# HKUST-Aerial-Robotics/FUEL

Hardware: NVIDIA H100
Metric: replans_per_sec (higher is better)
Workload: dtype f64 (cost/gradient), i32+f32 (ESDF), u8 (frontier)

## Files before the change

fuel_b200/csrc/frontier.cu:

```cuda
#include "common.cuh"

#include <cooperative_groups.h>

#include <algorithm>
#include <vector>

namespace cg = cooperative_groups;

namespace {

constexpr int NONE = 0x7fffffff;

struct FParams {
  int dom_lo[3], dom_n[3];
  int s_lo[3], s_hi[3];
  int z_min_idx;
  int cluster_min;
  double size_xy;
  float leaf, leaf_inv;
};

__device__ __forceinline__ int tri_at(const Geom& g, const uint8_t* __restrict__ occ, int x, int y,
                                      int z) {
  if (x < 0 || y < 0 || z < 0 || x >= g.nx || y >= g.ny || z >= g.nz) return -1;
// ... 962 lines not shown
  }
  if (threadIdx.x == 0) *n_new = carry;
}

__device__ __forceinline__ void relabel_item(Geom g, const int* __restrict__ k_addr, int* __restrict__ k_cl,
                               const ClusterMeta* __restrict__ meta, int K, int C_old, int _tid) {
  const int k = _tid;
  if (k >= K) return;
  const int c = k_cl[k];
  if (c >= C_old || !meta[c].do_split) return;
  if (cell_side(g, meta[c], k_addr[k]) == 1) k_cl[k] = meta[c].new_id;
}

__device__ __forceinline__ void clear_do_split_item(ClusterMeta* meta, int C, int _tid) {
  const int c = _tid;
  if (c < C) meta[c].do_split = 0;
}

__device__ __forceinline__ void init_meta_item(ClusterMeta* meta, int R, int _tid) {
  const int c = _tid;
  if (c >= R) return;
  ClusterMeta m;
  memset(&m, 0, sizeof(m));
  m.root = c;
  m.active = 1;
  meta[c] = m;
}

__global__ void init_parent_kernel(int* parent, int* claim, int* csize, int n) {
  init_parent_item(parent, claim, csize, n, blockIdx.x * blockDim.x + threadIdx.x);
}

__global__ void union_kernel(Geom g, const int* __restrict__ cell_addr,
                             const uint8_t* __restrict__ cell_cls, const int* __restrict__ cellidx,
                             int* parent, int n) {
  union_item(g, cell_addr, cell_cls, cellidx, parent, n, blockIdx.x * blockDim.x + threadIdx.x);
}

__global__ void flatten_kernel(int* parent, const uint8_t* __restrict__ cell_cls, int n) {
  flatten_item(parent, cell_cls, n, blockIdx.x * blockDim.x + threadIdx.x);
}

__global__ void claim_kernel(Geom g, FParams fp, const int* __restrict__ cell_addr,
                             const uint8_t* __restrict__ cell_cls, const int* __restrict__ cellidx,
                             const int* __restrict__ label, int* claim, int n) {
  claim_item(g, fp, cell_addr, cell_cls, cellidx, label, claim, n, blockIdx.x * blockDim.x + threadIdx.x);
}

__global__ void assign_kernel(const int* __restrict__ cell_addr, const uint8_t* __restrict__ cell_cls,
                              const int* __restrict__ label, const int* __restrict__ claim,
                              int* __restrict__ seed, int* csize, int8_t* __restrict__ flag, int n) {
  assign_item(cell_addr, cell_cls, label, claim, seed, csize, flag, n, blockIdx.x * blockDim.x + threadIdx.x);
}

__global__ void mark_kernel(const int* __restrict__ seed, const int* __restrict__ csize, int cluster_min,
                            int* __restrict__ is_root, int* __restrict__ is_kept, int n) {
  mark_item(seed, csize, cluster_min, is_root, is_kept, n, blockIdx.x * blockDim.x + threadIdx.x);
}

__global__ void reset_cellidx_kernel(const int* __restrict__ cell_addr, int* __restrict__ cellidx, int n) {
  reset_cellidx_item(cell_addr, cellidx, n, blockIdx.x * blockDim.x + threadIdx.x);
}

__global__ void gather_kept_kernel(const int* __restrict__ cell_addr, const int* __restrict__ seed,
                                   const int* __restrict__ is_kept, const int* __restrict__ kept_off,
                                   const int* __restrict__ root_rank, int* __restrict__ k_addr,
                                   int* __restrict__ k_cl, int* __restrict__ cellidx, int n) {
  gather_kept_item(cell_addr, seed, is_kept, kept_off, root_rank, k_addr, k_cl, cellidx, n, blockIdx.x * blockDim.x + threadIdx.x);
}

struct LevelCtl {
  const int* R;
  const int* K;
  int* n_new;
  int* c_final;
  int* ccur;
  int* cnext;
};

__global__ void stat_accum_kernel(Geom g, const int* __restrict__ k_addr, const int* __restrict__ k_cl,
                                  const ClusterMeta* __restrict__ meta, ClusterStat* st, LevelCtl ctl) {
  if (*ctl.n_new == 0) return;
  stat_accum_item(g, k_addr, k_cl, meta, st, *ctl.K, blockIdx.x * blockDim.x + threadIdx.x);
}

__global__ void downsample_kernel(Geom g, FParams fp, const int* __restrict__ k_addr,
                                  const int* __restrict__ k_cl, const int* __restrict__ cellidx,
                                  const ClusterMeta* __restrict__ meta, ClusterStat* st,
                                  float* __restrict__ k_cent, int* __restrict__ k_leaf, LevelCtl ctl) {
  if (*ctl.n_new == 0) return;
  downsample_item<true>(g, fp, k_addr, k_cl, cellidx, meta, st, k_cent, k_leaf, *ctl.K, blockIdx.x * blockDim.x + threadIdx.x);
}

__global__ void cov_kernel(Geom g, const int* __restrict__ k_cl, const int* __restrict__ k_leaf,
                           const float* __restrict__ k_cent, const ClusterMeta* __restrict__ meta,
                           ClusterStat* st, LevelCtl ctl) {
  if (*ctl.n_new == 0) return;
  cov_item<true>(g, k_cl, k_leaf, k_cent, meta, st, *ctl.K, blockIdx.x * blockDim.x + threadIdx.x);
}

__global__ void pca_kernel(Geom g, ClusterMeta* meta, const ClusterStat* __restrict__ st, LevelCtl ctl) {
  if (*ctl.n_new == 0) return;
  const int c = blockIdx.x * blockDim.x + threadIdx.x;
  mean_item(g, meta, st, *ctl.ccur, c);
  pca_item(meta, st, *ctl.ccur, c);
}

__global__ void side_count_kernel(Geom g, const int* __restrict__ k_addr, const int* __restrict__ k_cl,
                                  const ClusterMeta* __restrict__ meta, ClusterStat* st, LevelCtl ctl) {
  if (*ctl.n_new == 0) return;
  side_count_item(g, k_addr, k_cl, meta, st, *ctl.K, blockIdx.x * blockDim.x + threadIdx.x);
}

__global__ void __launch_bounds__(1024) split_alloc_kernel(ClusterMeta* meta, const ClusterStat* __restrict__ st,
                                                           LevelCtl ctl) {
  if (*ctl.n_new == 0) return;
  const int C = *ctl.ccur;
  __shared__ int made;
  split_alloc(meta, st, C, &made);
  __syncthreads();
  if (threadIdx.x == 0) {
    *ctl.cnext = C + made;
    *ctl.c_final = C + made;
    *ctl.n_new = made;
  }
}

__global__ void relabel_kernel(Geom g, const int* __restrict__ k_addr, int* __restrict__ k_cl,
                               const ClusterMeta* __restrict__ meta, LevelCtl ctl) {
  if (*ctl.n_new == 0) return;
  relabel_item(g, k_addr, k_cl, meta, *ctl.K, *ctl.ccur, blockIdx.x * blockDim.x + threadIdx.x);
}

__global__ void next_level_kernel(ClusterMeta* meta, ClusterStat* st, LevelCtl ctl) {
  if (*ctl.n_new == 0) return;
  const int c = blockIdx.x * blockDim.x + threadIdx.x;
  clear_do_split_item(meta, *ctl.ccur, c);
  stat_reset_item(st, meta, *ctl.cnext, c);
}

__global__ void init_meta_kernel(ClusterMeta* meta, ClusterStat* st, LevelCtl ctl) {
  const int R = *ctl.R;
  const int c = blockIdx.x * blockDim.x + threadIdx.x;
  init_meta_item(meta, R, c);
  stat_reset_item(st, meta, R, c);
  if (c == 0) {
    *ctl.ccur = R;
    *ctl.c_final = R;
    *ctl.n_new = (R > 0 && *ctl.K > 0) ? 1 : 0;
  }
}


constexpr int SMALL_CTAS = 8;
constexpr int SMALL_CAP = 32768;
constexpr int SMALL_CCAP = 8192;


__device__ __forceinline__ void mark_chunk_item(const int* __restrict__ seed, const int* __restrict__ csize, int cluster_min,
                                                int* __restrict__ root_mask, int* __restrict__ kept_mask, int n, int i) {
  bool kept = false, root = false;
  if (i < n) {
    const int s = seed[i];
    kept = s != NONE && csize[s] > cluster_min;
    root = kept && s == i;
  }
  const unsigned mk = __ballot_sync(0xffffffffu, kept), mr = __ballot_sync(0xffffffffu, root);
  if ((i & 31) == 0 && i < n) {
    kept_mask[i >> 5] = (int)mk;
    root_mask[i >> 5] = (int)mr;
  }
}
__device__ void chunk_scan_small(const int* __restrict__ root_mask, const int* __restrict__ kept_mask,
                                 int* __restrict__ root_off, int* __restrict__ kept_off, int nchunk,
                                 int* __restrict__ tot_root, int* __restrict__ tot_kept) {
  __shared__ unsigned wtot2[32];
  const int t = threadIdx.x, lane = t & 31, w = t >> 5;
  const unsigned v = t < nchunk ? ((unsigned)__popc((unsigned)root_mask[t]) << 16) + (unsigned)__popc((unsigned)kept_mask[t]) : 0u;
  unsigned inc = v;
#pragma unroll
  for (int o = 1; o < 32; o <<= 1) {
    const unsigned u = __shfl_up_sync(0xffffffffu, inc, o);
    if (lane >= o) inc += u;
  }
  if (lane == 31) wtot2[w] = inc;
  __syncthreads();
  if (w == 0) {
    const unsigned x = wtot2[lane];
    unsigned xi = x;
#pragma unroll
    for (int o = 1; o < 32; o <<= 1) {
      const unsigned u = __shfl_up_sync(0xffffffffu, xi, o);
      if (lane >= o) xi += u;
    }
    wtot2[lane] = xi - x;
    if (lane == 31) {
      *tot_root = (int)(xi >> 16);
      *tot_kept = (int)(xi & 0xffffu);
    }
  }
  __syncthreads();
  if (t < nchunk) {
    const unsigned ex = wtot2[w] + inc - v;
    root_off[t] = (int)(ex >> 16);
    kept_off[t] = (int)(ex & 0xffffu);
  }
}
__device__ __forceinline__ void gather_chunk_item(const int* __restrict__ cell_addr, const int* __restrict__ seed,
                                                  const int* __restrict__ kept_mask, const int* __restrict__ kept_off,
                                                  const int* __restrict__ root_mask, const int* __restrict__ root_off,
                                                  int* __restrict__ k_addr, int* __restrict__ k_cl,
                                                  int* __restrict__ cellidx, int n, int i) {
  if (i >= n) return;
  const unsigned mk = (unsigned)kept_mask[i >> 5];
  const int a = cell_addr[i];
  if ((mk >> (i & 31)) & 1u) {
    const int k = kept_off[i >> 5] + __popc(mk & ((1u << (i & 31)) - 1u));
    const int s = seed[i];
    k_addr[k] = a;
    k_cl[k] = root_off[s >> 5] + __popc((unsigned)root_mask[s >> 5] & ((1u << (s & 31)) - 1u));
    cellidx[a] = k;
  } else {
    cellidx[a] = -1;
  }
}

struct SmallBufs {
  int *cell_addr, *parent, *claim, *csize, *seed, *is_root, *is_kept, *root_rank, *kept_off;
  uint8_t* cell_cls;
  int *k_addr, *k_cl, *k_leaf;
  float* k_cent;
  ClusterMeta* meta;
  ClusterStat* stat;
  int* counters;
};

__global__ void __cluster_dims__(SMALL_CTAS, 1, 1) __launch_bounds__(1024) cluster_small_kernel(Geom g, FParams fp, int8_t* __restrict__ flag,
                                                             int* __restrict__ cellidx, SmallBufs b) {
  cg::cluster_group cluster = cg::this_cluster();
  const int rank = (int)cluster.block_rank();
  const int tid = (((int)threadIdx.x >> 5) * SMALL_CTAS + rank) * 32 + ((int)threadIdx.x & 31);
  constexpr int NT = 1024 * SMALL_CTAS;
  const int n = b.counters[0];
#ifdef FUEL_PROF
  long long* prof = (long long*)(b.counters + 8);
  int pi = 0;
#define STAMP() do { if (tid == 0) { long long t_; asm volatile("mov.u64 %0, %%globaltimer;" : "=l"(t_)); prof[pi++] = t_; } } while (0)
#else
#define STAMP() do {} while (0)
#endif
  STAMP();
  if (n > SMALL_CAP) {
    if (tid == 0) b.counters[4] = 1;
    return;
  }
#define FOR_ITEMS(i, N) for (int i = tid; i - tid < (N); i += NT)
  FOR_ITEMS(i, n) init_parent_item(b.parent, b.claim, b.csize, n, i);
  cluster.sync();
  STAMP();
  FOR_ITEMS(i, n) union_item(g, b.cell_addr, b.cell_cls, cellidx, b.parent, n, i);
  cluster.sync();
  STAMP();
  FOR_ITEMS(i, n) flatten_item(b.parent, b.cell_cls, n, i);
  cluster.sync();
  STAMP();
  FOR_ITEMS(i, n) claim_item(g, fp, b.cell_addr, b.cell_cls, cellidx, b.parent, b.claim, n, i);
  cluster.sync();
  STAMP();
  FOR_ITEMS(i, n) assign_item(b.cell_addr, b.cell_cls, b.parent, b.claim, b.seed, b.csize, flag, n, i);
  cluster.sync();
  STAMP();
  FOR_ITEMS(i, n) mark_chunk_item(b.seed, b.csize, fp.cluster_min, b.is_root, b.is_kept, n, i);
  cluster.sync();
  STAMP();
  if (rank == 0) chunk_scan_small(b.is_root, b.is_kept, b.root_rank, b.kept_off, (n + 31) >> 5, b.counters + 1, b.counters + 2);
  cluster.sync();
  STAMP();
  const int R = b.counters[1], K = b.counters[2];
  int C = R;
  int status = 0;
  if (R > 0 && K > 0) {
    FOR_ITEMS(i, n) gather_chunk_item(b.cell_addr, b.seed, b.is_kept, b.kept_off, b.is_root, b.root_rank, b.k_addr, b.k_cl,
                                      cellidx, n, i);
    FOR_ITEMS(c, R) {
      init_meta_item(b.meta, R, c);
      stat_reset_item(b.stat, b.meta, R, c);
    }
    cluster.sync();
    STAMP();
    for (int level = 0; level < 40; ++level) {
      if (2 * C > SMALL_CCAP) {
        status = 2;
        break;
      }
      FOR_ITEMS(k, K) stat_accum_item(g, b.k_addr, b.k_cl, b.meta, b.stat, K, k);
      cluster.sync();
      STAMP();
      FOR_ITEMS(c, C) mean_item(g, b.meta, b.stat, C, c);
      FOR_ITEMS(k, K) downsample_item<true>(g, fp, b.k_addr, b.k_cl, cellidx, b.meta, b.stat, b.k_cent, b.k_leaf, K, k);
      cluster.sync();
      STAMP();
      FOR_ITEMS(k, K) cov_item(g, b.k_cl, b.k_leaf, b.k_cent, b.meta, b.stat, K, k);
      cluster.sync();
      STAMP();
      FOR_ITEMS(c, C) pca_item(b.meta, b.stat, C, c);
      cluster.sync();
      STAMP();
      FOR_ITEMS(k, K) side_count_item(g, b.k_addr, b.k_cl, b.meta, b.stat, K, k);
      cluster.sync();
      STAMP();
      if (rank == 0) split_alloc(b.meta, b.stat, C, b.counters + 3);
      cluster.sync();
      STAMP();
      FOR_ITEMS(k, K) relabel_item(g, b.k_addr, b.k_cl, b.meta, K, C, k);
      cluster.sync();
      STAMP();
      const int n_new = b.counters[3];
      if (n_new == 0) break;
      FOR_ITEMS(c, C) clear_do_split_item(b.meta, C, c);
      C += n_new;
      FOR_ITEMS(c, C) stat_reset_item(b.stat, b.meta, C, c);
      cluster.sync();
      STAMP();
    }
  }
  FOR_ITEMS(i, n) reset_cellidx_item(b.cell_addr, cellidx, n, i);
  if (tid == 0) {
    b.counters[4] = status;
    b.counters[5] = C;
  }
#undef FOR_ITEMS
}

__global__ void is_changed_kernel(Geom g, const uint8_t* __restrict__ occ, const int* __restrict__ offs,
                                  const int* __restrict__ addr, uint8_t* __restrict__ changed, int* __restrict__ counts,
                                  int m) {
  const int c = blockIdx.x;
  if (c >= m) return;
  __shared__ int cnt;
  if (threadIdx.x == 0) cnt = 0;
  __syncthreads();
  int mine = 0;
  for (int i = offs[c] + threadIdx.x; i < offs[c + 1]; i += blockDim.x) {
    int x, y, z;
    addr_to_idx(g, addr[i], x, y, z);
    if (!frontier_pred(g, occ, x, y, z)) ++mine;
  }
  if (mine) atomicAdd(&cnt, mine);
  __syncthreads();
  if (threadIdx.x == 0) {
    if (changed) changed[c] = (uint8_t)(cnt > 0);
    if (counts) counts[c] = cnt;
  }
}

template <typename T>
struct DevBuf {
  T* p = nullptr;
  size_t cap = 0;
  int ensure(size_t n) {
    if (n <= cap) return 0;
    if (p) cudaFree(p);
    p = nullptr;
    cap = 0;
    size_t want = n + n / 4 + 1024;
    if (cudaMalloc(&p, want * sizeof(T)) != cudaSuccess) return FUELGPU_ENOMEM;
    cap = want;
    return 0;
  }
  int grow_preserve(size_t n, size_t keep, cudaStream_t s) {
    if (n <= cap) return 0;
    T* np = nullptr;
    size_t want = n + n / 2 + 1024;
    if (cudaMalloc(&np, want * sizeof(T)) != cudaSuccess) return FUELGPU_ENOMEM;
    if (p && keep) {
      cudaMemcpyAsync(np, p, keep * sizeof(T), cudaMemcpyDeviceToDevice, s);
      cudaStreamSynchronize(s);
    }
    if (p) cudaFree(p);
    p = np;
    cap = want;
    return 0;
  }
  void release() {
    if (p) cudaFree(p);
    p = nullptr;
    cap = 0;
  }
};

}

struct SweepPlan {
  bool words = false;
  unsigned nb = 0;
  size_t nmask = 0;
  int64_t ndom = 0;
  WordGeom wg;
};

struct HostView {
  const int *addr, *cl, *leaf;
  const float* cent;
  const ClusterMeta* meta;
  const ClusterStat* stat;
};

struct FrontierState {
  int* cellidx = nullptr;
  DevBuf<uint32_t> maskE, maskS;
  DevBuf<int> blockcnt, blockoff, scan_tot, scan_off;
  DevBuf<int> cell_addr, parent, claim, csize, seed, is_root, is_kept, root_rank, kept_off;
  DevBuf<uint8_t> cell_cls;
  DevBuf<int> k_addr, k_cl, k_leaf;
  DevBuf<float> k_cent;
  DevBuf<ClusterStat> stat;
  DevBuf<ClusterMeta> meta;
  bool small_ready = false;
  bool pend_active = false, pend_empty = true;
  FParams pend_fp;
  SweepPlan pend_plan;
  HostView pend_hv;
  cudaStream_t stream = nullptr;
  cudaEvent_t ev_in = nullptr;
  cudaEvent_t ev_out = nullptr;
  bool ev_out_valid = false;
  char* h_pin = nullptr;
  size_t h_pin_bytes = 0;
  int* d_counters = nullptr;
  std::vector<int32_t> h_cell_off, h_cell_addr, h_filt_off;
  std::vector<double> h_filtered, h_avg, h_bmin, h_bmax;
  int cell_order = FUELGPU_CELLS_BY_ADDRESS;
  float last_leaf = 0.f;
};

cudaStream_t frontier_stream_raw(FuelMap* m) { return m->fs->stream; }
cudaStream_t frontier_stream(FuelMap* m) {
  FrontierState* f = m->fs;
  cudaEventRecord(f->ev_in, m->stream);
  cudaStreamWaitEvent(f->stream, f->ev_in, 0);
  return f->stream;
}

int frontier_set_cell_order(FuelMap* m, int order) {
  if (order != FUELGPU_CELLS_BY_ADDRESS && order != FUELGPU_CELLS_BFS)
    return fuel_fail(m, FUELGPU_EINVAL, "unknown cell order");
  m->fs->cell_order = order;
  return 0;
}

void frontier_order_writer(FuelMap* m) {
  FrontierState* f = m->fs;
  if (f && f->ev_out_valid) cudaStreamWaitEvent(m->stream, f->ev_out, 0);
}

int frontier_state_create(FuelMap* m) {
  m->fs = new FrontierState();
  FUEL_CUDA(m, cudaStreamCreateWithFlags(&m->fs->stream, cudaStreamNonBlocking));
  FUEL_CUDA(m, cudaEventCreateWithFlags(&m->fs->ev_in, cudaEventDisableTiming));
  FUEL_CUDA(m, cudaEventCreateWithFlags(&m->fs->ev_out, cudaEventDisableTiming));
  FUEL_CUDA(m, cudaMalloc(&m->fs->cellidx, sizeof(int) * m->nvox));
  FUEL_CUDA(m, cudaMemsetAsync(m->fs->cellidx, 0xff, sizeof(int) * m->nvox, m->stream));
  FUEL_CUDA(m, cudaMalloc(&m->fs->d_counters, sizeof(int) * 8 + sizeof(long long) * 256));
  FUEL_CUDA(m, cudaMemsetAsync(m->fs->d_counters, 0, sizeof(int) * 8 + sizeof(long long) * 256, m->stream));
  return 0;
}

void frontier_state_destroy(FuelMap* m) {
  if (!m->fs) return;
  FrontierState* f = m->fs;
  if (f->cellidx) cudaFree(f->cellidx);
  if (f->d_counters) cudaFree(f->d_counters);
  if (f->h_pin) cudaFreeHost(f->h_pin);
  if (f->stream) {
    cudaStreamSynchronize(f->stream);
    cudaStreamDestroy(f->stream);
  }
  if (f->ev_in) cudaEventDestroy(f->ev_in);
  if (f->ev_out) cudaEventDestroy(f->ev_out);
  f->maskE.release(); f->maskS.release(); f->blockcnt.release(); f->blockoff.release();
  f->scan_tot.release(); f->scan_off.release();
  f->cell_addr.release(); f->parent.release(); f->claim.release(); f->csize.release();
  f->seed.release(); f->is_root.release(); f->is_kept.release(); f->root_rank.release();
  f->kept_off.release(); f->cell_cls.release(); f->k_addr.release(); f->k_cl.release();
  f->k_leaf.release(); f->k_cent.release(); f->stat.release(); f->meta.release();
  delete f;
  m->fs = nullptr;
}

#define ENSURE(buf, n)                                         \
  do {                                                         \
    if ((buf).ensure(n)) return fuel_fail(m, FUELGPU_ENOMEM, "frontier: device allocation failed"); \
  } while (0)

static inline unsigned nblk(int64_t n, int b) { return (unsigned)((n + b - 1) / b); }

static int scan_ints(FuelMap* m, const int* in, int* out, int n, int* total) {
  FrontierState* f = m->fs;
  cudaStream_t s = m->fs->stream;
  if (n <= 4096) {
    scan_kernel<<<1, 1024, 0, s>>>(in, out, n, total);
    FUEL_LAUNCHES(m, 1);
    return 0;
  }
  const int nchunk = (n + 1023) / 1024;
  if (f->scan_tot.ensure(nchunk) || f->scan_off.ensure(nchunk))
    return fuel_fail(m, FUELGPU_ENOMEM, "frontier: device allocation failed");
  scan_chunks_kernel<<<nchunk, 1024, 0, s>>>(in, out, n, f->scan_tot.p);
  scan_kernel<<<1, 1024, 0, s>>>(f->scan_tot.p, f->scan_off.p, nchunk, total);
  scan_add_kernel<<<nchunk, 1024, 0, s>>>(out, n, f->scan_off.p);
  FUEL_LAUNCHES(m, 3);
  return 0;
}

static SweepPlan sweep_plan(const Geom& g, const FParams& fp) {
  SweepPlan pl;
  pl.ndom = (int64_t)fp.dom_n[0] * fp.dom_n[1] * fp.dom_n[2];
  pl.words = (g.nz % 32) == 0 && pl.ndom > 0;
  if (pl.words) {
    const int z0 = fp.dom_lo[2], z1 = fp.dom_lo[2] + fp.dom_n[2] - 1;
    pl.wg.wz0 = z0 >> 5;
    pl.wg.NW = (z1 >> 5) - pl.wg.wz0 + 1;
    pl.wg.nwords = (int64_t)fp.dom_n[0] * fp.dom_n[1] * pl.wg.NW;
    pl.nb = nblk(pl.wg.nwords, WORD_BLOCK);
    pl.nmask = (size_t)pl.nb * WORD_BLOCK;
  } else {
    pl.nb = nblk(pl.ndom, CLS_BLOCK);
    pl.nmask = (size_t)pl.nb * (CLS_BLOCK / 32);
  }
  return pl;
}

static int sweep_classify(FuelMap* m, const FParams& fp, const SweepPlan& pl, cudaStream_t s) {
  FrontierState* f = m->fs;
  ENSURE(f->maskE, pl.nmask);
  ENSURE(f->maskS, pl.nmask);
  ENSURE(f->blockcnt, pl.nb);
  ENSURE(f->blockoff, pl.nb);
  if (pl.words)
    classify_words_kernel<<<pl.nb, WORD_BLOCK, 0, s>>>(m->g, fp, pl.wg, m->occ, m->flag, f->maskE.p, f->maskS.p,
                                                       f->blockcnt.p);
  else
    classify_kernel<<<pl.nb, CLS_BLOCK, 0, s>>>(m->g, fp, m->occ, m->flag, f->maskE.p, f->maskS.p, f->blockcnt.p,
                                                pl.ndom);
  FUEL_LAUNCHES(m, 1);
  if (scan_ints(m, f->blockcnt.p, f->blockoff.p, (int)pl.nb, f->d_counters + 0)) return FUELGPU_ENOMEM;
  return 0;
}

static void sweep_compact(FuelMap* m, const FParams& fp, const SweepPlan& pl, int* cellidx, int cap, cudaStream_t s) {
  FrontierState* f = m->fs;
  if (pl.words)
    compact_words_kernel<<<pl.nb, WORD_BLOCK, 0, s>>>(m->g, fp, pl.wg, f->maskE.p, f->maskS.p, f->blockoff.p,
                                                      f->cell_addr.p, f->cell_cls.p, cellidx, cap);
  else
    compact_kernel<<<pl.nb, CLS_BLOCK, 0, s>>>(m->g, fp, f->maskE.p, f->maskS.p, f->blockoff.p, f->cell_addr.p,
                                               f->cell_cls.p, cellidx, pl.ndom, cap);
  FUEL_LAUNCHES(m, 1);
}

static size_t view_bytes(int K, int C) {
  return (size_t)K * (3 * sizeof(int) + 3 * sizeof(float)) + (size_t)C * (sizeof(ClusterMeta) + sizeof(ClusterStat)) + 64;
}

static int ensure_pin(FuelMap* m, size_t bytes) {
  FrontierState* f = m->fs;
  if (bytes <= f->h_pin_bytes) return 0;
  if (f->h_pin) cudaFreeHost(f->h_pin);
  f->h_pin = nullptr;
  f->h_pin_bytes = 0;
  FUEL_CUDA(m, cudaMallocHost((void**)&f->h_pin, bytes));
  f->h_pin_bytes = bytes;
  return 0;
}

static int enqueue_download(FuelMap* m, int K, int C, char* base, HostView* v) {
  FrontierState* f = m->fs;
  cudaStream_t s = m->fs->stream;
  char* p = base;
  auto put = [&](const void* src, size_t bytes) -> char* {
    char* dst = p;
    p += (bytes + 15) & ~(size_t)15;
    if (bytes) cudaMemcpyAsync(dst, src, bytes, cudaMemcpyDeviceToHost, s);
    return dst;
  };
  v->meta = (const ClusterMeta*)put(f->meta.p, sizeof(ClusterMeta) * C);
  v->stat = (const ClusterStat*)put(f->stat.p, sizeof(ClusterStat) * C);
  v->addr = (const int*)put(f->k_addr.p, sizeof(int) * K);
  v->cl = (const int*)put(f->k_cl.p, sizeof(int) * K);
  v->leaf = (const int*)put(f->k_leaf.p, sizeof(int) * K);
  v->cent = (const float*)put(f->k_cent.p, sizeof(float) * 3 * K);
  FUEL_CUDA(m, cudaGetLastError());
  return 0;
}

static int frontier_build_csr(FuelMap* m, int K, int C, const HostView& hv, int32_t* n_clusters,
                              int32_t* n_cells, int32_t* n_filtered);

static void frontier_apply_bfs_order(FuelMap* m, const std::vector<int>& out_root) {
  FrontierState* f = m->fs;
  const Geom& g = m->g;
  const int C = (int)out_root.size();
  const int64_t sy = g.nz, sx = (int64_t)g.ny * g.nz;
  std::vector<int32_t> new_filt_off(C + 1, 0);
  std::vector<double> new_filtered;
  new_filtered.reserve(f->h_filtered.size());
  std::vector<int> tab;
  for (int r0 = 0; r0 < C;) {
    int r1 = r0 + 1;
    while (r1 < C && out_root[r1] == out_root[r0]) ++r1;
    const int a0 = f->h_cell_off[r0], a1 = f->h_cell_off[r1], n = a1 - a0;
    int cap = 16;
    while (cap < 2 * n) cap <<= 1;
    tab.assign(cap, -1);
    auto slot_of = [&](int addr) { return (int)(((uint32_t)addr * 2654435761u) & (uint32_t)(cap - 1)); };
    int seed = -1;
    const FParams& sp = f->pend_fp;
    for (int i = 0; i < n; ++i) {
      const int addr = f->h_cell_addr[a0 + i];
      const int cx = (int)(addr / sx), cy = (int)((addr % sx) / sy), cz = (int)(addr % sy);
      const bool in_search = cx >= sp.s_lo[0] && cx <= sp.s_hi[0] && cy >= sp.s_lo[1] && cy <= sp.s_hi[1] &&
                             cz >= sp.s_lo[2] && cz <= sp.s_hi[2];
      if (in_search && (seed < 0 || addr < f->h_cell_addr[a0 + seed])) seed = i;
      int s = slot_of(addr);
      while (tab[s] >= 0) s = (s + 1) & (cap - 1);
      tab[s] = i;
    }
    auto find = [&](int addr) {
      int s = slot_of(addr);
      while (tab[s] >= 0) {
        if (f->h_cell_addr[a0 + tab[s]] == addr) return tab[s];
        s = (s + 1) & (cap - 1);
      }
      return -1;
    };
    if (seed < 0) seed = 0;
    std::vector<int> bfs_rank(n, -1), queue;
    queue.reserve(n);
// ... 63 lines not shown
          for (int a = 0; a < 3; ++a) acc[a] += pf[(size_t)3 * lk[j].second + a];
          ++j;
        }
        const float cntf = (float)(j - i);
        for (int a = 0; a < 3; ++a) new_filtered.push_back((double)(acc[a] / cntf));
        ++nf;
        i = j;
      }
      new_filt_off[r + 1] = new_filt_off[r] + nf;
    }
    r0 = r1;
  }
  f->h_filt_off.swap(new_filt_off);
  f->h_filtered.swap(new_filtered);
}

static int frontier_marshal(FuelMap* m, int K, int C, int32_t* n_clusters, int32_t* n_cells,
                            int32_t* n_filtered) {
  int rc = ensure_pin(m, view_bytes(K, C));
  if (rc) return rc;
  HostView hv;
  rc = enqueue_download(m, K, C, m->fs->h_pin, &hv);
  if (rc) return rc;
  FUEL_CUDA(m, cudaStreamSynchronize(m->fs->stream));
  return frontier_build_csr(m, K, C, hv, n_clusters, n_cells, n_filtered);
}

static int frontier_build_csr(FuelMap* m, int K, int C, const HostView& hv, int32_t* n_clusters,
                              int32_t* n_cells, int32_t* n_filtered) {
  FrontierState* f = m->fs;
  const Geom& g = m->g;
  const int* h_addr = hv.addr;
  const int* h_cl = hv.cl;
  const int* h_leaf = hv.leaf;
  const float* h_cent = hv.cent;
  const ClusterMeta* h_meta = hv.meta;
  const ClusterStat* h_stat = hv.stat;
  std::vector<int> order(C);
  for (int c = 0; c < C; ++c) order[c] = c;
  std::sort(order.begin(), order.end(), [&](int a, int b) {
    if (h_meta[a].root != h_meta[b].root) return h_meta[a].root < h_meta[b].root;
    return h_meta[a].path < h_meta[b].path;
  });
  std::vector<int> rank(C);
  for (int i = 0; i < C; ++i) rank[order[i]] = i;

  f->h_cell_off.assign(C + 1, 0);
  f->h_filt_off.assign(C + 1, 0);
  for (int k = 0; k < K; ++k) {
    f->h_cell_off[rank[h_cl[k]] + 1]++;
    if (h_leaf[k] >= 0) f->h_filt_off[rank[h_cl[k]] + 1]++;
  }
  for (int c = 0; c < C; ++c) {
    f->h_cell_off[c + 1] += f->h_cell_off[c];
    f->h_filt_off[c + 1] += f->h_filt_off[c];
  }
  f->h_cell_addr.resize(K);
  const int NF = f->h_filt_off[C];
  std::vector<std::pair<int, int>> filt_keys(NF);
  {
    std::vector<int> cur(f->h_cell_off.begin(), f->h_cell_off.end() - 1);
    std::vector<int> curf(f->h_filt_off.begin(), f->h_filt_off.end() - 1);
    for (int k = 0; k < K; ++k) {
      const int r = rank[h_cl[k]];
      f->h_cell_addr[cur[r]++] = h_addr[k];
      if (h_leaf[k] >= 0) filt_keys[curf[r]++] = std::make_pair(h_leaf[k], k);
    }
  }
  f->h_filtered.resize((size_t)3 * NF);
  for (int c = 0; c < C; ++c) {
    std::sort(filt_keys.begin() + f->h_filt_off[c], filt_keys.begin() + f->h_filt_off[c + 1]);
    for (int i = f->h_filt_off[c]; i < f->h_filt_off[c + 1]; ++i) {
      const int k = filt_keys[i].second;
      for (int a = 0; a < 3; ++a) f->h_filtered[(size_t)3 * i + a] = (double)h_cent[(size_t)3 * k + a];
    }
  }
  f->h_avg.resize((size_t)3 * C);
  f->h_bmin.resize((size_t)3 * C);
  f->h_bmax.resize((size_t)3 * C);
  for (int c = 0; c < C; ++c) {
    const int r = rank[c];
    for (int a = 0; a < 3; ++a) {
      f->h_avg[(size_t)3 * r + a] = h_meta[c].mean[a];
      f->h_bmin[(size_t)3 * r + a] = (h_stat[c].lo[a] + 0.5) * g.res + g.origin[a];
      f->h_bmax[(size_t)3 * r + a] = (h_stat[c].hi[a] + 0.5) * g.res + g.origin[a];
    }
  }
  *n_clusters = C;
  *n_cells = K;
  *n_filtered = NF;
  if (f->cell_order == FUELGPU_CELLS_BFS) {
    std::vector<int> out_root(C);
    for (int c = 0; c < C; ++c) out_root[rank[c]] = h_meta[c].root;
    frontier_apply_bfs_order(m, out_root);
    *n_filtered = f->h_filt_off[C];
  }
  return 0;
}

static int frontier_cluster_large(FuelMap* m, const FParams& fp, int n_cand, int32_t* n_clusters, int32_t* n_cells,
                                  int32_t* n_filtered);

static void frontier_make_params(FuelMap* m, const double umin[3], const double umax[3], const FuelFrontierParams* p,
                                 FParams* out) {
  FrontierState* f = m->fs;
  const Geom& g = m->g;
  const int nmax[3] = { g.nx, g.ny, g.nz };
  FParams fp;
  const double infl[3] = { 1, 1, 0.5 };
  for (int k = 0; k < 3; ++k) {
    double lo = umin[k] - infl[k], hi = umax[k] + infl[k];
    lo = lo > g.box_mind[k] ? lo : g.box_mind[k];
    hi = hi < g.box_maxd[k] ? hi : g.box_maxd[k];
    int ilo = (int)floor((lo - g.origin[k]) * g.res_inv);
    int ihi = (int)floor((hi - g.origin[k]) * g.res_inv);
    fp.s_lo[k] = ilo < 0 ? 0 : ilo;
    fp.s_hi[k] = ihi > nmax[k] - 1 ? nmax[k] - 1 : ihi;
    int dlo = g.box_min[k] < fp.s_lo[k] ? g.box_min[k] : fp.s_lo[k];
    int dhi = g.box_max[k] > fp.s_hi[k] ? g.box_max[k] : fp.s_hi[k];
    dlo = dlo < 0 ? 0 : dlo;
    dhi = dhi > nmax[k] - 1 ? nmax[k] - 1 : dhi;
    fp.dom_lo[k] = dlo;
    fp.dom_n[k] = dhi - dlo + 1;
    if (fp.dom_n[k] <= 0) {
      fp.dom_n[k] = 0;
    }
  }
  {
    int zi = 0;
    while (zi < g.nz && ((zi + 0.5) * g.res + g.origin[2]) < p->min_z) ++zi;
    fp.z_min_idx = zi;
  }
  fp.cluster_min = p->cluster_min;
  fp.size_xy = p->cluster_size_xy;
  fp.leaf = (float)(g.res * p->down_sample);
  f->last_leaf = fp.leaf;
  fp.leaf_inv = 1.0f / fp.leaf;
  f->pend_fp = fp;
  *out = fp;
}

static void frontier_clear_results(FrontierState* f) {
  f->h_cell_off.assign(1, 0);
  f->h_cell_addr.clear();
  f->h_filt_off.assign(1, 0);
  f->h_filtered.clear();
  f->h_avg.clear();
  f->h_bmin.clear();
  f->h_bmax.clear();
  f->pend_active = false;
  f->pend_empty = true;
}

int frontier_search_begin_impl(FuelMap* m, const double umin[3], const double umax[3],
                               const FuelFrontierParams* p) {
  FrontierState* f = m->fs;
  const Geom& g = m->g;
  cudaStream_t s = m->fs->stream;
  FParams fp;
  frontier_make_params(m, umin, umax, p, &fp);

  f->h_cell_off.assign(1, 0);
  f->h_cell_addr.clear();
  f->h_filt_off.assign(1, 0);
  f->h_filtered.clear();
  f->h_avg.clear();
  f->h_bmin.clear();
  f->h_bmax.clear();
  f->pend_active = false;
  f->pend_empty = true;

  const SweepPlan pl = sweep_plan(g, fp);
  if (pl.ndom <= 0) return 0;
  f->pend_empty = false;
  {
    const int rc = sweep_classify(m, fp, pl, s);
    if (rc) return rc;
  }
  {
    ENSURE(f->cell_addr, SMALL_CAP); ENSURE(f->cell_cls, SMALL_CAP); ENSURE(f->parent, SMALL_CAP);
    ENSURE(f->claim, SMALL_CAP); ENSURE(f->csize, SMALL_CAP); ENSURE(f->seed, SMALL_CAP);
    ENSURE(f->is_root, SMALL_CAP); ENSURE(f->is_kept, SMALL_CAP); ENSURE(f->root_rank, SMALL_CAP);
    ENSURE(f->kept_off, SMALL_CAP); ENSURE(f->k_addr, SMALL_CAP); ENSURE(f->k_cl, SMALL_CAP);
    ENSURE(f->k_leaf, SMALL_CAP); ENSURE(f->k_cent, (size_t)3 * SMALL_CAP);
    ENSURE(f->meta, SMALL_CCAP); ENSURE(f->stat, SMALL_CCAP);
    sweep_compact(m, fp, pl, f->cellidx, SMALL_CAP, s);
    SmallBufs sb;
    sb.cell_addr = f->cell_addr.p; sb.parent = f->parent.p; sb.claim = f->claim.p; sb.csize = f->csize.p;
    sb.seed = f->seed.p; sb.is_root = f->is_root.p; sb.is_kept = f->is_kept.p; sb.root_rank = f->root_rank.p;
    sb.kept_off = f->kept_off.p; sb.cell_cls = f->cell_cls.p; sb.k_addr = f->k_addr.p; sb.k_cl = f->k_cl.p;
    sb.k_leaf = f->k_leaf.p; sb.k_cent = f->k_cent.p; sb.meta = f->meta.p; sb.stat = f->stat.p;
    sb.counters = f->d_counters;
    cluster_small_kernel<<<SMALL_CTAS, 1024, 0, s>>>(g, fp, m->flag, f->cellidx, sb);
    FUEL_LAUNCHES(m, 1);
    constexpr int K0 = 12288, C0 = 256;
    int rc0 = ensure_pin(m, 64 + view_bytes(K0, C0));
    if (rc0) return rc0;
    int* cnt = (int*)f->h_pin;
    FUEL_CUDA(m, cudaMemcpyAsync(cnt, f->d_counters, sizeof(int) * 8, cudaMemcpyDeviceToHost, s));
    HostView& hv = f->pend_hv;
    rc0 = enqueue_download(m, K0, C0, f->h_pin + 64, &hv);
    if (rc0) return rc0;
    f->pend_fp = fp;
    f->pend_plan = pl;
    f->pend_active = true;
  }
  cudaEventRecord(f->ev_out, f->stream);
  f->ev_out_valid = true;
  return 0;
}

int frontier_search_end_impl(FuelMap* m, int32_t* n_clusters, int32_t* n_cells, int32_t* n_filtered) {
  FrontierState* f = m->fs;
  const Geom& g = m->g;
  cudaStream_t s = m->fs->stream;
  *n_clusters = *n_cells = *n_filtered = 0;
  if (f->pend_empty || !f->pend_active) {
    f->pend_active = false;
    return 0;
  }
  f->pend_active = false;
  const FParams fp = f->pend_fp;
  const SweepPlan pl = f->pend_plan;
  int n_cand = 0;
  {
    constexpr int K0 = 12288, C0 = 256;
    int* cnt = (int*)f->h_pin;
    HostView& hv = f->pend_hv;
    FUEL_CUDA(m, cudaStreamSynchronize(s));
    n_cand = cnt[0];
    if (n_cand == 0) return 0;
    if (cnt[4] == 0) {
      const int R = cnt[1], K = cnt[2], C = cnt[5];
      if (R == 0 || K == 0) return 0;
      if (K <= K0 && C <= C0) return frontier_build_csr(m, K, C, hv, n_clusters, n_cells, n_filtered);
      return frontier_marshal(m, K, C, n_clusters, n_cells, n_filtered);
    }
    if (cnt[4] == 1) {
      reset_cellidx_kernel<<<nblk(SMALL_CAP, 256), 256, 0, s>>>(f->cell_addr.p, f->cellidx, SMALL_CAP);
      FUEL_LAUNCHES(m, 1);
    }
  }

  ENSURE(f->cell_addr, n_cand); ENSURE(f->cell_cls, n_cand); ENSURE(f->parent, n_cand);
  ENSURE(f->claim, n_cand); ENSURE(f->csize, n_cand); ENSURE(f->seed, n_cand);
  ENSURE(f->is_root, n_cand); ENSURE(f->is_kept, n_cand); ENSURE(f->root_rank, n_cand);
  ENSURE(f->kept_off, n_cand);

  sweep_compact(m, fp, pl, f->cellidx, n_cand, s);
  return frontier_cluster_large(m, fp, n_cand, n_clusters, n_cells, n_filtered);
}

static int frontier_cluster_large(FuelMap* m, const FParams& fp, int n_cand, int32_t* n_clusters, int32_t* n_cells,
                                  int32_t* n_filtered) {
  FrontierState* f = m->fs;
  const Geom& g = m->g;
  cudaStream_t s = m->fs->stream;
  ENSURE(f->parent, n_cand);
  ENSURE(f->claim, n_cand); ENSURE(f->csize, n_cand); ENSURE(f->seed, n_cand);
  ENSURE(f->is_root, n_cand); ENSURE(f->is_kept, n_cand); ENSURE(f->root_rank, n_cand);
  ENSURE(f->kept_off, n_cand);
  ENSURE(f->k_addr, n_cand); ENSURE(f->k_cl, n_cand); ENSURE(f->k_leaf, n_cand); ENSURE(f->k_cent, (size_t)3 * n_cand);
  ENSURE(f->meta, (size_t)n_cand + 1024);
  ENSURE(f->stat, (size_t)n_cand + 1024);
  const unsigned cb = nblk(n_cand, 256);
  init_parent_kernel<<<cb, 256, 0, s>>>(f->parent.p, f->claim.p, f->csize.p, n_cand);
  union_kernel<<<cb, 256, 0, s>>>(g, f->cell_addr.p, f->cell_cls.p, f->cellidx, f->parent.p, n_cand);
  flatten_kernel<<<cb, 256, 0, s>>>(f->parent.p, f->cell_cls.p, n_cand);
  claim_kernel<<<cb, 256, 0, s>>>(g, fp, f->cell_addr.p, f->cell_cls.p, f->cellidx, f->parent.p, f->claim.p, n_cand);
  assign_kernel<<<cb, 256, 0, s>>>(f->cell_addr.p, f->cell_cls.p, f->parent.p, f->claim.p, f->seed.p,
                                   f->csize.p, m->flag, n_cand);
  mark_kernel<<<cb, 256, 0, s>>>(f->seed.p, f->csize.p, fp.cluster_min, f->is_root.p, f->is_kept.p, n_cand);
  FUEL_LAUNCHES(m, 6);
  if (scan_ints(m, f->is_root.p, f->root_rank.p, n_cand, f->d_counters + 1)) return FUELGPU_ENOMEM;
  if (scan_ints(m, f->is_kept.p, f->kept_off.p, n_cand, f->d_counters + 2)) return FUELGPU_ENOMEM;
  gather_kept_kernel<<<cb, 256, 0, s>>>(f->cell_addr.p, f->seed.p, f->is_kept.p, f->kept_off.p,
                                        f->root_rank.p, f->k_addr.p, f->k_cl.p, f->cellidx, n_cand);
  FUEL_LAUNCHES(m, 1);

  LevelCtl ctl;
  ctl.R = f->d_counters + 1;
  ctl.K = f->d_counters + 2;
  ctl.n_new = f->d_counters + 3;
  ctl.c_final = f->d_counters + 5;
  ctl.ccur = f->d_counters + 6;
  ctl.cnext = f->d_counters + 7;
  const int64_t r_ub = n_cand / ((fp.cluster_min > 0 ? fp.cluster_min : 0) + 1) + 1;
  init_meta_kernel<<<nblk(r_ub, 256), 256, 0, s>>>(f->meta.p, f->stat.p, ctl);
  FUEL_LAUNCHES(m, 1);
  int cnt[8] = { 0, 0, 0, 0, 0, 0, 0, 0 };
  constexpr int LEVELS_PER_BATCH = 12, MAX_LEVELS = 36;
  auto c_bound = [&](int level) -> int64_t {
    const int64_t c = level < 24 ? (r_ub << level) : (int64_t)n_cand;
    return c > n_cand ? (int64_t)n_cand : c;
  };
  for (int level = 0; level < MAX_LEVELS; ++level) {
    const unsigned ccb = nblk(c_bound(level), 256);
    stat_accum_kernel<<<cb, 256, 0, s>>>(g, f->k_addr.p, f->k_cl.p, f->meta.p, f->stat.p, ctl);
    downsample_kernel<<<cb, 256, 0, s>>>(g, fp, f->k_addr.p, f->k_cl.p, f->cellidx, f->meta.p, f->stat.p,
                                         f->k_cent.p, f->k_leaf.p, ctl);
    cov_kernel<<<cb, 256, 0, s>>>(g, f->k_cl.p, f->k_leaf.p, f->k_cent.p, f->meta.p, f->stat.p, ctl);
    pca_kernel<<<ccb, 256, 0, s>>>(g, f->meta.p, f->stat.p, ctl);
    side_count_kernel<<<cb, 256, 0, s>>>(g, f->k_addr.p, f->k_cl.p, f->meta.p, f->stat.p, ctl);
    split_alloc_kernel<<<1, 1024, 0, s>>>(f->meta.p, f->stat.p, ctl);
    relabel_kernel<<<cb, 256, 0, s>>>(g, f->k_addr.p, f->k_cl.p, f->meta.p, ctl);
    next_level_kernel<<<nblk(c_bound(level + 1), 256), 256, 0, s>>>(f->meta.p, f->stat.p, ctl);
    FUEL_LAUNCHES(m, 8);
    int* t = ctl.ccur;
    ctl.ccur = ctl.cnext;
    ctl.cnext = t;
    if ((level + 1) % LEVELS_PER_BATCH == 0 || level + 1 == MAX_LEVELS) {
      FUEL_CUDA(m, cudaMemcpyAsync(cnt, f->d_counters, sizeof(int) * 8, cudaMemcpyDeviceToHost, s));
      FUEL_CUDA(m, cudaStreamSynchronize(s));
      if (cnt[3] == 0) break;
    }
  }
  reset_cellidx_kernel<<<cb, 256, 0, s>>>(f->cell_addr.p, f->cellidx, n_cand);
  FUEL_LAUNCHES(m, 1);
  FUEL_CUDA(m, cudaGetLastError());
  const int R = cnt[1], K = cnt[2], C = cnt[5];
  if (R == 0 || K == 0) return 0;
  return frontier_marshal(m, K, C, n_clusters, n_cells, n_filtered);
}


__global__ void set_cellidx_kernel(const int* __restrict__ cell_addr, int* __restrict__ cellidx, int n) {
  const int i = blockIdx.x * blockDim.x + threadIdx.x;
  if (i < n) cellidx[cell_addr[i]] = i;
}

int frontier_candidates_impl(FuelMap* m, const double umin[3], const double umax[3], const FuelFrontierParams* p, int z_lo,
                             int z_hi, int32_t* n_out) {
  FrontierState* f = m->fs;
  const Geom& g = m->g;
  cudaStream_t s = frontier_stream(m);
  FParams fp;
  frontier_make_params(m, umin, umax, p, &fp);
  *n_out = 0;
  const int dz0 = fp.dom_lo[2] > z_lo ? fp.dom_lo[2] : z_lo;
  const int dz1 = (fp.dom_lo[2] + fp.dom_n[2] - 1) < z_hi ? (fp.dom_lo[2] + fp.dom_n[2] - 1) : z_hi;
  if (dz1 < dz0) return 0;
  fp.dom_lo[2] = dz0;
  fp.dom_n[2] = dz1 - dz0 + 1;
  const SweepPlan pl = sweep_plan(g, fp);
  if (pl.ndom <= 0) return 0;
  {
// ... 117 lines not shown
```

Measured before the change: 2059.

## Fuse split-level phases, double-buffer stats, and allow 16-CTA non-portable clusters

Restructures the per-level split loop in the clustered small kernel. Per-level stats are double-buffered so the next level's accumulation is fused into relabel. PCA is folded into side counting, and split allocation becomes a redundant per-CTA shared-memory scan, cutting several cluster.sync barriers per level. It also launches with a 16-CTA non-portable cluster when occupancy allows, falling back to 8. This adds warp-level match/reduce aggregation and redundant per-thread PCA, and relies on every CTA computing identical split ids.

```diff
diff --git a/fuel_b200/csrc/frontier.cu b/fuel_b200/csrc/frontier.cu
--- a/fuel_b200/csrc/frontier.cu
+++ b/fuel_b200/csrc/frontier.cu
@@ -1138,7 +1138,7 @@
 }
 
 
-constexpr int SMALL_CTAS = 8;
+constexpr int SMALL_CTAS_MAX = 16, SMALL_CTAS_PORTABLE = 8;
 constexpr int SMALL_CAP = 32768;
 constexpr int SMALL_CCAP = 8192;
 
@@ -1211,6 +1211,136 @@
   }
 }
 
+__device__ __forceinline__ void stat_clear_item(ClusterStat* st, int C, int _tid) {
+  const int c = _tid;
+  if (c >= C) return;
+  ClusterStat s;
+  memset(&s, 0, sizeof(s));
+  s.lo[0] = s.lo[1] = s.lo[2] = NONE;
+  s.hi[0] = s.hi[1] = s.hi[2] = -1;
+  st[c] = s;
+}
+
+__device__ __forceinline__ void stat_add_cell(ClusterStat* st, int c, int x, int y, int z) {
+  const unsigned grp = __match_any_sync(__activemask(), c);
+  if (c < 0) return;
+  const int sx = __reduce_add_sync(grp, x), sy = __reduce_add_sync(grp, y), sz = __reduce_add_sync(grp, z);
+  const int lx = __reduce_min_sync(grp, x), ly = __reduce_min_sync(grp, y), lz = __reduce_min_sync(grp, z);
+  const int hx = __reduce_max_sync(grp, x), hy = __reduce_max_sync(grp, y), hz = __reduce_max_sync(grp, z);
+  if ((int)(threadIdx.x & 31) != __ffs(grp) - 1) return;
+  ClusterStat* s = &st[c];
+  atomicAdd((unsigned long long*)&s->sx, (unsigned long long)sx);
+  atomicAdd((unsigned long long*)&s->sy, (unsigned long long)sy);
+  atomicAdd((unsigned long long*)&s->sz, (unsigned long long)sz);
+  atomicAdd(&s->n, __popc(grp));
+  atomicMin(&s->lo[0], lx);
+  atomicMin(&s->lo[1], ly);
+  atomicMin(&s->lo[2], lz);
+  atomicMax(&s->hi[0], hx);
+  atomicMax(&s->hi[1], hy);
+  atomicMax(&s->hi[2], hz);
+}
+
+__device__ __noinline__ double2 principal_axis_v(double a, double b, double d) {
+  double pc[2];
+  principal_axis_2x2(a, b, d, pc);
+  return make_double2(pc[0], pc[1]);
+}
+__device__ __forceinline__ void side_count_pca_item(Geom g, const int* __restrict__ k_addr, const int* __restrict__ k_cl,
+                                                    const ClusterMeta* meta, ClusterStat* st, int K, int _tid) {
+  const int k = _tid;
+  int c = -1, side = 0;
+  if (k < K) {
+    c = k_cl[k];
+    const ClusterStat& s = st[c];
+    if (!meta[c].active || !s.need_split || meta[c].depth >= 32) {
+      c = -1;
+    } else {
+      const double m = (double)s.nfilt;
+      const double cxx = fx_get(s.cxx_hi, s.cxx_lo) / m, cxy = fx_get(s.cxy_hi, s.cxy_lo) / m,
+                   cyy = fx_get(s.cyy_hi, s.cyy_lo) / m;
+      ClusterMeta mt;
+      mt.mean[0] = meta[c].mean[0];
+      mt.mean[1] = meta[c].mean[1];
+      const double2 pc = principal_axis_v(cxx, cxy, cyy);
+      mt.pc[0] = pc.x; mt.pc[1] = pc.y;
+      side = cell_side(g, mt, k_addr[k]);
+    }
+  }
+  const unsigned grp = __match_any_sync(__activemask(), c);
+  if (c < 0) return;
+  const int n1 = __reduce_add_sync(grp, side);
+  if ((int)(threadIdx.x & 31) != __ffs(grp) - 1) return;
+  const int n0 = __popc(grp) - n1;
+  if (n0) atomicAdd(&st[c].cnt0, n0);
+  if (n1) atomicAdd(&st[c].cnt1, n1);
+}
+
+__device__ int split_alloc_shared(ClusterMeta* meta, const ClusterStat* lvl, ClusterStat* fin, int C, int* nid,
+                                  bool writer) {
+  __shared__ int wsum[32];
+  const int lane = (int)threadIdx.x & 31, w = (int)threadIdx.x >> 5;
+  int carry = 0;
+  for (int base = 0; base < C; base += 1024) {
+    const int c = base + (int)threadIdx.x;
+    const bool v = c < C && lvl[c].cnt0 > 0 && lvl[c].cnt1 > 0;
+    const unsigned bal = __ballot_sync(0xffffffffu, v);
+    if (lane == 0) wsum[w] = __popc(bal);
+    __syncthreads();
+    int ex = carry + __popc(bal & ((1u << lane) - 1u)), tot = carry;
+#pragma unroll
+    for (int q = 0; q < 32; ++q) {
+      const int s = wsum[q];
+      tot += s;
+      if (q < w) ex += s;
+    }
+    if (c < C) {
+      nid[c] = v ? C + ex : -1;
+      if (writer && v) {
+        ClusterMeta& p = meta[c];
+        ClusterMeta ch = p;
+        p.new_id = C + ex;
+        ch.path = p.path | (1u << (31 - p.depth));
+        ch.depth = p.depth + 1;
+        ch.active = 1;
+        ch.do_split = 0;
+        p.depth += 1;
+        p.do_split = 0;
+        meta[C + ex] = ch;
+      } else if (writer && meta[c].active) {
+        meta[c].do_split = 0;
+        meta[c].active = 0;
+        fin[c] = lvl[c];
+      }
+    }
+    carry = tot;
+    __syncthreads();
+  }
+  return carry;
+}
+
+__device__ __forceinline__ void relabel_accum_item(Geom g, const int* __restrict__ k_addr, int* __restrict__ k_cl,
+                                                   const ClusterMeta* meta, const int* nid, ClusterStat* st_next, int K,
+                                                   int _tid) {
+  const int k = _tid;
+  int c = -1, x = 0, y = 0, z = 0;
+  if (k < K) {
+    c = k_cl[k];
+    const int id = nid[c];
+    if (id < 0) {
+      c = -1;
+    } else {
+      const int a = k_addr[k];
+      if (cell_side(g, meta[c], a) == 1) {
+        k_cl[k] = id;
+        c = id;
+      }
+      addr_to_idx(g, a, x, y, z);
+    }
+  }
+  stat_add_cell(st_next, c, x, y, z);
+}
+
 struct SmallBufs {
   int *cell_addr, *parent, *claim, *csize, *seed, *is_root, *is_kept, *root_rank, *kept_off;
   uint8_t* cell_cls;
@@ -1218,10 +1348,12 @@
   float* k_cent;
   ClusterMeta* meta;
   ClusterStat* stat;
+  ClusterStat* lvl;
   int* counters;
 };
 
-__global__ void __cluster_dims__(SMALL_CTAS, 1, 1) __launch_bounds__(1024) cluster_small_kernel(Geom g, FParams fp, int8_t* __restrict__ flag,
+template <int SMALL_CTAS>
+__global__ void __launch_bounds__(1024) cluster_small_kernel(Geom g, FParams fp, int8_t* __restrict__ flag,
                                                              int* __restrict__ cellidx, SmallBufs b) {
   cg::cluster_group cluster = cg::this_cluster();
   const int rank = (int)cluster.block_rank();
@@ -1264,14 +1396,18 @@
   STAMP();
   const int R = b.counters[1], K = b.counters[2];
   int C = R;
-  int status = 0;
+  int status = 0, n_new = 0;
   if (R > 0 && K > 0) {
+    __shared__ int nid[SMALL_CCAP / 2];
     FOR_ITEMS(i, n) gather_chunk_item(b.cell_addr, b.seed, b.is_kept, b.kept_off, b.is_root, b.root_rank, b.k_addr, b.k_cl,
                                       cellidx, n, i);
     FOR_ITEMS(c, R) {
       init_meta_item(b.meta, R, c);
-      stat_reset_item(b.stat, b.meta, R, c);
-    }
+      stat_clear_item(b.lvl, R, c);
+    }
+    cluster.sync();
+    STAMP();
+    FOR_ITEMS(k, K) stat_accum_item(g, b.k_addr, b.k_cl, b.meta, b.lvl, K, k);
     cluster.sync();
     STAMP();
     for (int level = 0; level < 40; ++level) {
@@ -1279,39 +1415,31 @@
         status = 2;
         break;
       }
-      FOR_ITEMS(k, K) stat_accum_item(g, b.k_addr, b.k_cl, b.meta, b.stat, K, k);
+      ClusterStat* const st = b.lvl + (level & 1) * SMALL_CCAP;
+      ClusterStat* const st_next = b.lvl + ((level & 1) ^ 1) * SMALL_CCAP;
+      FOR_ITEMS(c, C) mean_item(g, b.meta, st, C, c);
+      FOR_ITEMS(k, K) downsample_item<true>(g, fp, b.k_addr, b.k_cl, cellidx, b.meta, st, b.k_cent, b.k_leaf, K, k);
+      FOR_ITEMS(c, 2 * C) stat_clear_item(st_next, 2 * C, c);
       cluster.sync();
       STAMP();
-      FOR_ITEMS(c, C) mean_item(g, b.meta, b.stat, C, c);
-      FOR_ITEMS(k, K) downsample_item<true>(g, fp, b.k_addr, b.k_cl, cellidx, b.meta, b.stat, b.k_cent, b.k_leaf, K, k);
+      FOR_ITEMS(k, K) cov_item(g, b.k_cl, b.k_leaf, b.k_cent, b.meta, st, K, k);
       cluster.sync();
       STAMP();
-      FOR_ITEMS(k, K) cov_item(g, b.k_cl, b.k_leaf, b.k_cent, b.meta, b.stat, K, k);
+      FOR_ITEMS(c, C) pca_item(b.meta, st, C, c);
+      FOR_ITEMS(k, K) side_count_pca_item(g, b.k_addr, b.k_cl, b.meta, st, K, k);
       cluster.sync();
       STAMP();
-      FOR_ITEMS(c, C) pca_item(b.meta, b.stat, C, c);
+      n_new = split_alloc_shared(b.meta, st, b.stat, C, nid, rank == 0);
+      if (n_new == 0) break;
+      FOR_ITEMS(k, K) relabel_accum_item(g, b.k_addr, b.k_cl, b.meta, nid, st_next, K, k);
+      C += n_new;
       cluster.sync();
       STAMP();
-      FOR_ITEMS(k, K) side_count_item(g, b.k_addr, b.k_cl, b.meta, b.stat, K, k);
-      cluster.sync();
-      STAMP();
-      if (rank == 0) split_alloc(b.meta, b.stat, C, b.counters + 3);
-      cluster.sync();
-      STAMP();
-      FOR_ITEMS(k, K) relabel_item(g, b.k_addr, b.k_cl, b.meta, K, C, k);
-      cluster.sync();
-      STAMP();
-      const int n_new = b.counters[3];
-      if (n_new == 0) break;
-      FOR_ITEMS(c, C) clear_do_split_item(b.meta, C, c);
-      C += n_new;
-      FOR_ITEMS(c, C) stat_reset_item(b.stat, b.meta, C, c);
-      cluster.sync();
-      STAMP();
     }
   }
   FOR_ITEMS(i, n) reset_cellidx_item(b.cell_addr, cellidx, n, i);
   if (tid == 0) {
+    b.counters[3] = n_new;
     b.counters[4] = status;
     b.counters[5] = C;
   }
@@ -1401,8 +1529,10 @@
   DevBuf<int> k_addr, k_cl, k_leaf;
   DevBuf<float> k_cent;
   DevBuf<ClusterStat> stat;
+  DevBuf<ClusterStat> lvl_stat;
   DevBuf<ClusterMeta> meta;
   bool small_ready = false;
+  int small_ctas = 0;
   bool pend_active = false, pend_empty = true;
   FParams pend_fp;
   SweepPlan pend_plan;
@@ -1469,7 +1599,7 @@
   f->cell_addr.release(); f->parent.release(); f->claim.release(); f->csize.release();
   f->seed.release(); f->is_root.release(); f->is_kept.release(); f->root_rank.release();
   f->kept_off.release(); f->cell_cls.release(); f->k_addr.release(); f->k_cl.release();
-  f->k_leaf.release(); f->k_cent.release(); f->stat.release(); f->meta.release();
+  f->k_leaf.release(); f->k_cent.release(); f->stat.release(); f->lvl_stat.release(); f->meta.release();
   delete f;
   m->fs = nullptr;
 }
@@ -1839,6 +1969,36 @@
   f->pend_empty = true;
 }
 
+static void small_cluster_config(int ctas, cudaStream_t s, cudaLaunchConfig_t* cfg, cudaLaunchAttribute* attr) {
+  cfg->gridDim = dim3(ctas, 1, 1);
+  cfg->blockDim = dim3(1024, 1, 1);
+  cfg->dynamicSmemBytes = 0;
+  cfg->stream = s;
+  attr->id = cudaLaunchAttributeClusterDimension;
+  attr->val.clusterDim.x = ctas;
+  attr->val.clusterDim.y = 1;
+  attr->val.clusterDim.z = 1;
+  cfg->attrs = attr;
+  cfg->numAttrs = 1;
+}
+
+static int small_cluster_ctas(FrontierState* f) {
+  if (f->small_ctas) return f->small_ctas;
+  f->small_ctas = SMALL_CTAS_PORTABLE;
+  if (cudaFuncSetAttribute(cluster_small_kernel<SMALL_CTAS_MAX>, cudaFuncAttributeNonPortableClusterSizeAllowed, 1) ==
+      cudaSuccess) {
+    cudaLaunchConfig_t cfg = {};
+    cudaLaunchAttribute attr;
+    small_cluster_config(SMALL_CTAS_MAX, f->stream, &cfg, &attr);
+    int nclusters = 0;
+    if (cudaOccupancyMaxActiveClusters(&nclusters, cluster_small_kernel<SMALL_CTAS_MAX>, &cfg) == cudaSuccess &&
+        nclusters > 0)
+      f->small_ctas = SMALL_CTAS_MAX;
+  }
+  cudaGetLastError();
+  return f->small_ctas;
+}
+
 int frontier_search_begin_impl(FuelMap* m, const double umin[3], const double umax[3],
                                const FuelFrontierParams* p) {
   FrontierState* f = m->fs;
@@ -1870,15 +2030,24 @@
     ENSURE(f->is_root, SMALL_CAP); ENSURE(f->is_kept, SMALL_CAP); ENSURE(f->root_rank, SMALL_CAP);
     ENSURE(f->kept_off, SMALL_CAP); ENSURE(f->k_addr, SMALL_CAP); ENSURE(f->k_cl, SMALL_CAP);
     ENSURE(f->k_leaf, SMALL_CAP); ENSURE(f->k_cent, (size_t)3 * SMALL_CAP);
-    ENSURE(f->meta, SMALL_CCAP); ENSURE(f->stat, SMALL_CCAP);
+    ENSURE(f->meta, SMALL_CCAP); ENSURE(f->stat, SMALL_CCAP); ENSURE(f->lvl_stat, 2 * SMALL_CCAP);
     sweep_compact(m, fp, pl, f->cellidx, SMALL_CAP, s);
     SmallBufs sb;
     sb.cell_addr = f->cell_addr.p; sb.parent = f->parent.p; sb.claim = f->claim.p; sb.csize = f->csize.p;
     sb.seed = f->seed.p; sb.is_root = f->is_root.p; sb.is_kept = f->is_kept.p; sb.root_rank = f->root_rank.p;
     sb.kept_off = f->kept_off.p; sb.cell_cls = f->cell_cls.p; sb.k_addr = f->k_addr.p; sb.k_cl = f->k_cl.p;
     sb.k_leaf = f->k_leaf.p; sb.k_cent = f->k_cent.p; sb.meta = f->meta.p; sb.stat = f->stat.p;
+    sb.lvl = f->lvl_stat.p;
     sb.counters = f->d_counters;
-    cluster_small_kernel<<<SMALL_CTAS, 1024, 0, s>>>(g, fp, m->flag, f->cellidx, sb);
+    {
+      const int ctas = small_cluster_ctas(f);
+      cudaLaunchConfig_t cfg = {};
+      cudaLaunchAttribute attr;
+      small_cluster_config(ctas, s, &cfg, &attr);
+      FUEL_CUDA(m, cudaLaunchKernelEx(&cfg, ctas == SMALL_CTAS_MAX ? cluster_small_kernel<SMALL_CTAS_MAX>
+                                                                   : cluster_small_kernel<SMALL_CTAS_PORTABLE>,
+                                      g, fp, m->flag, f->cellidx, sb));
+    }
     FUEL_LAUNCHES(m, 1);
     constexpr int K0 = 12288, C0 = 256;
     int rc0 = ensure_pin(m, 64 + view_bytes(K0, C0));
```

New measurement: 2396 (median of 6 runs). +16.4%, better.
